# Arieys/MonteCarloPathTracing

Measured on AMD Instinct MI355X. Metric: Mrays/s on cornell-box 1280x720 SPP=256 (closest-hit queries actually traced / wall time incl. gather), higher is better.
Workload: dtype f64

## Files before the change

montecarlopathtracing_amd/csrc/camera.hip:

```cpp
#include <hip/hip_runtime.h>

#include "camera.hpp"
#include "dev_common.hpp"
#include "kernels.hpp"
#include "shade_common.hpp"
#include "shade_path.hpp"
#include "vertex.hpp"
#include "wavefront.hpp"

namespace mcpt {

__global__ void k_primary_pos(DCamera cam, double* __restrict__ pos_out)
{
    const int row = blockIdx.x * blockDim.x + threadIdx.x;
    if (row >= cam.height) return;
    const V3 pdx = ld3(cam.pdx);
    V3 pos = ld3(cam.start_point) - ld3(cam.pdy) * (double)row;
    double* out = pos_out + (size_t)row * cam.width * 3;
    for (int j = 0; j < cam.width; j++) {
        out[j * 3] = pos.x; out[j * 3 + 1] = pos.y; out[j * 3 + 2] = pos.z;
        pos = pos + pdx;
    }
}

// ... 76 lines not shown
    stc(a.out.bdir, cap, j, d);
    a.out.btype[j] = RT_TRANSMISSION | MCPT_BT_NO_OFFSET;
    for (int l = 0; l < a.nl; l++) a.out.expect[(long long)l * cap + j] = -2;
}

template <bool PROG, bool ENV>
__global__ void k_fold_lens(const double* __restrict__ rad, const uint8_t* __restrict__ flags, const int32_t* __restrict__ pixels, int first_slot,
                            int n_slots, int n, int k0, int N, double* __restrict__ img, double* __restrict__ mom, uint8_t* __restrict__ hit,
                            int32_t* __restrict__ hitcnt)
{
    const long long gid = (long long)blockIdx.x * blockDim.x + threadIdx.x;
    if (gid >= (long long)n_slots * 3) return;
    const int s = (int)(gid / 3), c = (int)(gid % 3);
    const int slot = first_slot + s;
    const int pix = pixels ? pixels[slot] : slot;
    const double* src = rad + (size_t)s * n * 3 + c;
    const uint8_t* f = flags + (size_t)s * n;
    int h = 0;
    for (int k = 0; k < n; k++) h += f[k];
    const size_t i = (size_t)pix * 3 + c;
    if (!PROG) {
        float acc = 0.0f;
        if (h > 0 || ENV)
            for (int k = 0; k < n; k++) acc = (float)((double)acc + src[(size_t)k * 3] / n);
        img[i] = (double)acc;
        return;
    }
    if (c == 0) {
        const int total = (k0 > 0 ? hitcnt[pix] : 0) + h;
        hitcnt[pix] = total;
        hit[pix] = total > 0 ? 1 : 0;
    }
    double* m = mom + (size_t)pix * 6 + c;
    if (h == 0 && !ENV) {
        if (k0 == 0) { img[i] = 0.0; m[0] = 0.0; m[3] = 0.0; }
        return;
    }
    float acc = k0 > 0 ? (float)img[i] : 0.0f;
    double s1 = k0 > 0 ? m[0] : 0.0, s2 = k0 > 0 ? m[3] : 0.0;
    for (int k = 0; k < n; k++) {
        const double x = src[(size_t)k * 3];
        acc = (float)((double)acc + x / N);
        s1 += x;
        s2 += x * x;
    }
    img[i] = (double)acc;
    m[0] = s1; m[3] = s2;
}

template <bool ENV>
__global__ void k_fold_motion(const double* __restrict__ rad, const int32_t* __restrict__ pixels, const PrimaryHit* __restrict__ hits, int first_slot,
                              int n_slots, int n, int k0, int N, double* __restrict__ img, double* __restrict__ mom, uint8_t* __restrict__ hit, DEnv env,
                              const double* __restrict__ dirs)
{
    const long long gid = (long long)blockIdx.x * blockDim.x + threadIdx.x;
    if (gid >= (long long)n_slots * 3) return;
    const int s = (int)(gid / 3), c = (int)(gid % 3);
    const int slot = first_slot + s;
    const int pix = pixels ? pixels[slot] : slot;
    const bool h = hits[slot].leaf >= 0;
    if (c == 0) hit[pix] = (uint8_t)((k0 > 0 ? hit[pix] : 0) | (h ? 1 : 0));
    const size_t i = (size_t)pix * 3 + c;
    double* m = mom + (size_t)pix * 6 + c;
    double le = 0.0;
    if (!h) {
        if (ENV) {
            const V3 e = env_eval(env, ld3(dirs + (size_t)pix * 3));
            le = c == 0 ? e.x : (c == 1 ? e.y : e.z);
        } else {
            if (k0 == 0) { img[i] = 0.0; m[0] = 0.0; m[3] = 0.0; }
            return;
        }
    }
    const double* src = rad + (size_t)s * n * 3 + c;
    float acc = k0 > 0 ? (float)img[i] : 0.0f;
    double s1 = k0 > 0 ? m[0] : 0.0, s2 = k0 > 0 ? m[3] : 0.0;
    for (int k = 0; k < n; k++) {
        const double x = h ? src[(size_t)k * 3] : le;
        acc = (float)((double)acc + x / N);
        s1 += x;
        s2 += x * x;
    }
    img[i] = (double)acc;
    m[0] = s1; m[3] = s2;
}

static inline unsigned blocks_of(long long n, int block) { return (unsigned)((n + block - 1) / block); }

void launch_primary_pos(const DCamera& cam, double* d_pos, hipStream_t st)
{
    hipLaunchKernelGGL(k_primary_pos, dim3(blocks_of(cam.height, 64)), dim3(64), 0, st, cam, d_pos);
}
void launch_camera_rays(const DLens& lens, unsigned long long seed, const int32_t* d_pix, const int32_t* d_k, long long n, double* d_rays6, hipStream_t st)
{
    if (n <= 0) return;
    hipLaunchKernelGGL(k_camera_rays, dim3(blocks_of(n, 256)), dim3(256), 0, st, lens, seed, d_pix, d_k, n, d_rays6);
}
void launch_shade_samples_lens(const DScene& S, const DLens& lens, unsigned long long seed, const int32_t* d_pixels, int first_slot, int n_slots, int spp,
                               int sample_base, double* d_rad, uint8_t* d_flags, DCounters* ctr, hipStream_t st)
{
    const long long n = (long long)n_slots * spp;
    if (n <= 0) return;
    const dim3 grid(blocks_of(n, 256));
    with_path_variant(S, [&](auto env, auto pick) {
        hipLaunchKernelGGL((k_shade_samples_lens<env(), pick()>), grid, dim3(256), 0, st, S, lens, seed, d_pixels, first_slot, n, spp, sample_base, d_rad, d_flags, ctr);
// ... 40 lines not shown
```

montecarlopathtracing_amd/csrc/dev_common.hpp:

```cpp
#pragma once
#include <hip/hip_runtime.h>

#include "device_scene.hpp"

namespace mcpt {

#define MCPT_PI 3.1415926
#define MCPT_P_RR 0.6

struct V3 { double x, y, z; };
__device__ __forceinline__ V3 mk(double x, double y, double z) { V3 r; r.x = x; r.y = y; r.z = z; return r; }
__device__ __forceinline__ V3 ld3(const double* p) { return mk(p[0], p[1], p[2]); }
__device__ __forceinline__ V3 operator+(V3 a, V3 b) { return mk(a.x + b.x, a.y + b.y, a.z + b.z); }
__device__ __forceinline__ V3 operator-(V3 a, V3 b) { return mk(a.x - b.x, a.y - b.y, a.z - b.z); }
__device__ __forceinline__ V3 operator*(V3 a, double t) { return mk(a.x * t, a.y * t, a.z * t); }
__device__ __forceinline__ V3 operator/(V3 a, double m) { return mk(a.x / m, a.y / m, a.z / m); }
__device__ __forceinline__ V3 mul(V3 a, V3 b) { return mk(a.x * b.x, a.y * b.y, a.z * b.z); }
__device__ __forceinline__ V3 neg(V3 a) { return mk(-a.x, -a.y, -a.z); }
__device__ __forceinline__ double dot(V3 a, V3 b) { return a.x * b.x + a.y * b.y + a.z * b.z; }
__device__ __forceinline__ V3 cross(V3 a, V3 b) { return mk(a.y * b.z - b.y * a.z, b.x * a.z - a.x * b.z, a.x * b.y - b.x * a.y); }
__device__ __forceinline__ double norm(V3 a) { return sqrt(a.x * a.x + a.y * a.y + a.z * a.z); }
__device__ __forceinline__ V3 normalized(V3 a) { double d = norm(a); return mk(a.x / d, a.y / d, a.z / d); }

__device__ __forceinline__ V3 ldc(const double* __restrict__ a, long long cap, long long i)
// ... 166 lines not shown
    for (int off = 32; off > 0; off >>= 1) { unsigned int o = __shfl_down(v, off, 64); v = o > v ? o : v; }
    return v;
}
struct LaneStats { uint32_t nodes = 0, tris = 0, shadow = 0, bounce = 0, primary = 0, shades = 0, samples = 0, depth = 0, skipped = 0; };
__device__ __forceinline__ void flush_stats(DCounters* c, const LaneStats& s)
{
    if (!c) return;
    const unsigned long long n = wave_sum(s.nodes), t = wave_sum(s.tris), sh = wave_sum(s.shadow), bo = wave_sum(s.bounce),
                             pr = wave_sum(s.primary), sc = wave_sum(s.shades), sa = wave_sum(s.samples), sk = wave_sum(s.skipped);
    const unsigned int md = wave_max(s.depth);
    if ((threadIdx.x & 63) == 0) {
        if (n) atomicAdd(&c->node_visits, n);
        if (t) atomicAdd(&c->tri_tests, t);
        if (sh) atomicAdd(&c->rays_shadow, sh);
        if (bo) atomicAdd(&c->rays_bounce, bo);
        if (pr) atomicAdd(&c->rays_primary, pr);
        if (sc) atomicAdd(&c->shade_calls, sc);
        if (sa) atomicAdd(&c->samples, sa);
        if (sk) atomicAdd(&c->shadow_skipped, sk);
        if (md) atomicMax(&c->max_depth, (unsigned long long)md);
    }
}


}
```

montecarlopathtracing_amd/csrc/kernels.hip:

```cpp
#include <hip/hip_runtime.h>

#include "accel_build.hpp"
#include "dev_common.hpp"
#include "kernels.hpp"
#include "shade_common.hpp"
#include "shade_path.hpp"
#include "trace_persistent.hpp"
#include "trace_pool.hpp"

namespace mcpt {

template <bool LEAF>
__global__ void __launch_bounds__(256) k_trace_closest_reference(DScene S, const double* __restrict__ rays, long long n,
                                                       int32_t* __restrict__ face, double* __restrict__ t_out,
                                                       double* __restrict__ p_out, double* __restrict__ pn_out, DCounters* ctr)
{
    const long long gid = (long long)blockIdx.x * blockDim.x + threadIdx.x;
    LaneStats ls;
    if (gid < n) {
        Ray r;
        r.o = ld3(rays + gid * 6); r.d = ld3(rays + gid * 6 + 3);
        Hit h; Work w = {0, 0};
        const bool ok = trace_closest(S, r, h, w);
        ls.nodes = w.nodes; ls.tris = w.tris; ls.primary = 1;
// ... 196 lines not shown
__global__ void __launch_bounds__(256) k_light_pick_at(DLightPick pick, int nl, unsigned long long seed, const int32_t* __restrict__ pix, const int32_t* __restrict__ ks,
                                                       int depth, const double* __restrict__ p, const double* __restrict__ pn, long long n,
                                                       int32_t* __restrict__ light, double* __restrict__ pdf)
{
    const long long gid = (long long)blockIdx.x * blockDim.x + threadIdx.x;
    if (gid >= n) return;
    RngKey key; key.k0 = (uint32_t)seed; key.k1 = (uint32_t)(seed >> 32); key.pixel = (uint32_t)pix[gid]; key.sample = (uint32_t)ks[gid];
    double q;
    light[gid] = light_pick_at(pick, key, (uint32_t)depth, (uint32_t)nl, ld3(p + gid * 3), ld3(pn + gid * 3), q);
    pdf[gid] = q;
}

template <bool ENV>
__global__ void k_fold_samples(const double* __restrict__ rad, const int32_t* __restrict__ pixels, const PrimaryHit* __restrict__ hits,
                               int first_slot, int n_slots, int spp, double* __restrict__ img, DEnv env, const double* __restrict__ dirs)
{
    const long long gid = (long long)blockIdx.x * blockDim.x + threadIdx.x;
    if (gid >= (long long)n_slots * 3) return;
    const int s = (int)(gid / 3), c = (int)(gid % 3);
    const double* src = rad + (size_t)s * spp * 3 + c;
    const int slot = first_slot + s;
    float acc = 0.0f;
    if (hits[slot].leaf >= 0)
        for (int k = 0; k < spp; k++) acc = (float)((double)acc + src[(size_t)k * 3] / spp);
    else if (ENV) {
        const V3 le = env_eval(env, ld3(dirs + (size_t)(pixels ? pixels[slot] : slot) * 3));
        const double x = c == 0 ? le.x : (c == 1 ? le.y : le.z);
        for (int k = 0; k < spp; k++) acc = (float)((double)acc + x / spp);
    }
    const int pix = pixels ? pixels[slot] : slot;
    img[(size_t)pix * 3 + c] = (double)acc;
}

template <bool ENV>
__global__ void k_fold_progressive(const double* __restrict__ rad, const int32_t* __restrict__ pixels, const PrimaryHit* __restrict__ hits,
                                   int first_slot, int n_slots, int n, int k0, int N, double* __restrict__ img, double* __restrict__ mom,
                                   uint8_t* __restrict__ hit, DEnv env, const double* __restrict__ dirs)
{
    const long long gid = (long long)blockIdx.x * blockDim.x + threadIdx.x;
    if (gid >= (long long)n_slots * 3) return;
    const int s = (int)(gid / 3), c = (int)(gid % 3);
    const int slot = first_slot + s;
    const int pix = pixels ? pixels[slot] : slot;
    const bool h = hits[slot].leaf >= 0;
    if (c == 0) hit[pix] = h ? 1 : 0;
    if (!h) {
        if (ENV) {
            const V3 le = env_eval(env, ld3(dirs + (size_t)pix * 3));
            const double x = c == 0 ? le.x : (c == 1 ? le.y : le.z);
            double* m = mom + (size_t)pix * 6 + c;
            float acc = 0.0f;
            for (int k = 0; k < N; k++) acc = (float)((double)acc + x / N);
            double s1 = k0 > 0 ? m[0] : 0.0;
            for (int k = 0; k < n; k++) s1 += x;
            img[(size_t)pix * 3 + c] = (double)acc;
            m[0] = s1; m[3] = 0.0;
        } else img[(size_t)pix * 3 + c] = 0.0;
        return;
    }
    const double* src = rad + (size_t)s * n * 3 + c;
    double* m = mom + (size_t)pix * 6 + c;
    float acc = k0 > 0 ? (float)img[(size_t)pix * 3 + c] : 0.0f;
    double s1 = k0 > 0 ? m[0] : 0.0, s2 = k0 > 0 ? m[3] : 0.0;
    for (int k = 0; k < n; k++) {
        const double x = src[(size_t)k * 3];
        acc = (float)((double)acc + x / N);
        s1 += x;
        s2 += x * x;
    }
    img[(size_t)pix * 3 + c] = (double)acc;
    m[0] = s1; m[3] = s2;
}

__device__ __forceinline__ double wave_sum_fixed(double v)
{
    for (int o = 32; o >= 1; o >>= 1) v += __shfl_xor(v, o, 64);
    return v;
}
__device__ __forceinline__ void block_sum3(double v[3], double* out)
{
    __shared__ double part[4][3];
    const int w = threadIdx.x >> 6, lane = threadIdx.x & 63;
    for (int i = 0; i < 3; i++) v[i] = wave_sum_fixed(v[i]);
    if (lane == 0) for (int i = 0; i < 3; i++) part[w][i] = v[i];
    __syncthreads();
    if (threadIdx.x == 0)
        for (int i = 0; i < 3; i++) out[i] = ((part[0][i] + part[1][i]) + part[2][i]) + part[3][i];
}
template <bool PER_PIXEL>
__global__ void __launch_bounds__(256) k_noise_reduce(const int32_t* __restrict__ pixels, long long n_pixels, long long per_range,
                                                      const double* __restrict__ mom, const uint8_t* __restrict__ hit, int done,
                                                      const int32_t* __restrict__ cnt, double* __restrict__ partials)
// ... 313 lines not shown
```

montecarlopathtracing_amd/csrc/render.cpp:

```cpp
#include <hip/hip_runtime_api.h>

#include <algorithm>
#include <cmath>
#include <cstdio>
#include <cstring>
#include <functional>
#include <string>
#include <vector>

#include "handles.hpp"

using namespace mcpt;

int ensure_dirs(mcpt_device* d, hipStream_t st)
{
    if (!d->dirs_ready) {
        launch_primary_dirs(d->ds.cam, d->dirs.get(), st);
        HIP_TRY(hipGetLastError());
        HIP_TRY(hipStreamSynchronize(st));
        d->dirs_ready = true;
    }
    return MCPT_OK;
}

// ... 156 lines not shown
    int64_t chunk_slots = std::max<int64_t>(cap / spp, 1);
    chunk_slots = std::min<int64_t>(chunk_slots, npx);
    cap = chunk_slots * spp;
    const size_t ws_need = size_t(cap) * bpp + overhead;
    HIP_TRY(f.wf_ws.grow_bytes(ws_need));
    HIP_TRY(f.rad.grow_bytes(size_t(cap) * 3 * sizeof(double)));
    if (per_sample) {
        HIP_TRY(f.cam_hit.grow(size_t(cap)));
    } else {
        HIP_TRY(f.hit_slots.grow(size_t(chunk_slots)));
        HIP_TRY(f.surf.grow(size_t(chunk_slots)));
        HIP_TRY(f.alive_base.grow(size_t(chunk_slots / 64 + 2)));
    }
    int rc = MCPT_OK;
    WfArgs a{};
    WfState A, B;
    if (!wf_carve(f.wf_ws.get(), f.wf_ws.bytes(), cap, nl, A, B, a.rays)) return fail(MCPT_ERR_NOMEM, "wavefront workspace too small");
    char* path_area = f.path_area.get();
    if (nl != S.num_lights && d->cfg.finish_pool) {
        const size_t need = finish_pool_bytes(d->cfg.cus, nl);
        if (!need) path_area = nullptr;
        else { HIP_TRY(f.path_area.grow_bytes(need)); path_area = f.path_area.get(); }
    }
    a.cap = cap; a.nl = nl; a.spp = spp; a.sample_base = r.k0; a.seed = p->seed; a.pixels = L.pixels; a.hit_slots = f.hit_slots.get(); a.surf = f.surf.get(); a.alive_base = f.alive_base.get();
    a.hits = f.hits.get(); a.dirs = d->dirs.get(); a.rad = f.rad.get(); a.counts = f.wf_counts.get(); a.ctr = f.ctr.get(); a.tris = d->tris.get();
    a.materials = d->materials.get(); a.queue = fast ? f.queue.get() : nullptr;
    a.finish_below = fast ? unsigned(std::min<long long>(std::max<long long>(d->finish_threshold, 0), 1ll << 30)) : 0u;
    if (per_sample) { a.hits = nullptr; a.cam_hit = f.cam_hit.get(); }
    const size_t ev_first = d->ev_used;
    const int kSyncEvery = 4;
    for (int64_t first = 0; first < npx; first += chunk_slots) {
        const int n_slots = int(std::min<int64_t>(chunk_slots, npx - first));
        HIP_TRY(hipMemsetAsync(f.wf_counts.get(), 0, sizeof(WfCounts) * MCPT_WF_COUNT_SLOTS, st));
        long long n_upper = (long long)n_slots * spp;
        double n_grid = double(n_upper);
        a.first_slot = int(first);
        a.in = A; a.out = B;
        a.counts_in = &f.wf_counts[0];
        if (per_sample) {
            WfArgs ac = a;
            ac.depth = -1; ac.counts = &f.wf_counts[0]; ac.count_mul = 1u; ac.finish_below = 0u;
            if (src.query) launch_query_pass(*src.query, ac, n_upper, st);
            else launch_camera_pass(*src.lens, ac, n_upper, st);
            HIP_TRY(hipGetLastError());
            ac.nl = 0;
            EventPair* pr = nullptr;
            if (timed || keep) { if ((rc = next_pair(d->ev_pool, d->ev_used, pr))) return rc; HIP_TRY(hipEventRecord(pr->first.get(), st)); }
// ... 294 lines not shown
```

montecarlopathtracing_amd/csrc/trace_pool.hpp:

```cpp
#pragma once
#include "env.hpp"
#include "trace_persistent.hpp"
#include "vertex.hpp"

namespace mcpt {

struct NoPaths { static constexpr bool kPaths = false; };

#ifndef MCPT_POOL_WAVES
#define MCPT_POOL_WAVES 16
#endif
#ifndef MCPT_POOL_KT
#define MCPT_POOL_KT 20
#endif
#ifndef MCPT_POOL_STACK
#define MCPT_POOL_STACK 8
#endif
#define MCPT_POOL_SPILL (MCPT_FAST_STACK - MCPT_POOL_STACK)
#ifndef MCPT_POOL_CLAIMS
#define MCPT_POOL_CLAIMS 2
#endif
#define MCPT_POOL_CLAIM_ORDER __ATOMIC_ACQUIRE
#define MCPT_POOL_FILE_ORDER __ATOMIC_RELEASE

// ... 427 lines not shown
                }
                const bool want_path = have && mode == P_FREE;
                const unsigned long long wb = __ballot(want_path);
                bool dead = false;
                if (wb) {
                    long long mine = pp.n;
                    if (!queue_empty) {
                        const unsigned int want = (unsigned int)__popcll(wb);
                        unsigned int got = 0;
                        if (lane == 0) got = atomicAdd(&a.counts->finish_claimed, want);
                        got = (unsigned int)uni((int)got);
                        if ((long long)got + want >= pp.n) queue_empty = true;
                        mine = (long long)got + (int)__builtin_amdgcn_mbcnt_hi((unsigned int)(wb >> 32), __builtin_amdgcn_mbcnt_lo((unsigned int)wb, 0u));
                    }
                    if (want_path) {
                        if (mine < pp.n) {
                            const long long j = mine;
                            id = a.out.id[j];
                            depth = (uint32_t)a.depth;
                            T = mk(1, 1, 1); Lr = mk(0, 0, 0);
                            if (folded && a.depth == 0) { const int b0 = a.out.btype[j]; if (b0 >= 0) T = first_vertex_throughput(S, a, id, b0); }
                            else if (a.depth > 0 || folded) T = ldc(a.out.T, cap, j);
                            if (a.depth > 0) Lr = ldc(a.out.L, cap, j);
                            if (a.depth == 0) { const PrimaryHit* ph = a.hits + (a.first_slot + id / a.spp); p = mk(ph->p[0], ph->p[1], ph->p[2]); }
                            else p = ldc(a.out.p, cap, j);
                            for (int l = 0; l < nl; l++) {
                                const int expect = a.out.expect[(long long)l * cap + j];
                                ri[(size_t)(RI_EXPECT + l) * plane] = expect;
                                if (expect != -2) {
                                    const V3 cc = ldc(a.out.c + (long long)l * 3 * cap, cap, j), d = ldc(a.rays.d + (long long)l * 3 * cap, cap, j);
                                    stp(RD_C + 3 * l, cc); emit(s0 + l, p + d * 0.01, d);
                                }
                            }
                            const int bt = a.out.btype[j];
                            ri[RI_BT * plane] = bt;
                            if (bt >= 0) {
                                const V3 bd = ldc(a.out.bdir, cap, j);
                                if (!folded) stp(RD_W, ldc(a.out.w, cap, j));
                                emit(s0 + nl, (bt & MCPT_BT_NO_OFFSET) ? p : p + bd * 0.01, bd);
                            }
                            ri[RI_ID * plane] = id; ri[RI_DEPTH * plane] = (int)depth;
                            stp(RD_T, T); stp(RD_L, Lr);
                            mode = P_ADOPTED;
                        } else dead = true;
                    }
                }
                if (have) {
// ... 143 lines not shown
```

montecarlopathtracing_amd/csrc/vertex.hpp:

```cpp
#pragma once
#include "dev_common.hpp"
#include "shade_common.hpp"
#include "light_tree.hpp"
#include "wavefront.hpp"

namespace mcpt {

__device__ __forceinline__ V3 after_bounce(const V3& T, const V3& wgt)
{
    return mk(T.x * wgt.x * MCPT_INV_P_RR, T.y * wgt.y * MCPT_INV_P_RR, T.z * wgt.z * MCPT_INV_P_RR);
}
__device__ __forceinline__ V3 first_vertex_throughput(const DScene& S, const WfArgs& a, int id, int bt)
{
    const PrimarySurface* ps = a.surf + a.hits[a.first_slot + id / a.spp].surf;
    const int type = bt & 7;
    const V3 wgt = type == RT_DIFFUSE ? ld3(ps->kd) : (type == RT_SPECULAR ? ld3(S.materials[ps->material].ks) : mk(1, 1, 1));
    return after_bounce(mk(1, 1, 1), wgt);
}
__device__ __forceinline__ void add_if_visible(V3& L_dir, const V3& c, bool vis)
{
    L_dir.x += vis ? c.x : c.x * 0.0;
    L_dir.y += vis ? c.y : c.y * 0.0;
    L_dir.z += vis ? c.z : c.z * 0.0;
}
struct PathLights { int nplanes, nlights; bool folded; };
template <bool ENV, int PICK>
__device__ __forceinline__ PathLights path_lights(const DScene& S, int nl)
{
    const int nplanes = ENV ? nl - 1 : nl;
    return {nplanes, PICK ? S.num_lights : nplanes, nl == 1};
}
__device__ __forceinline__ RngKey sample_key(const WfArgs& a, int id, int pixel)
{
    RngKey key;
    key.k0 = (uint32_t)a.seed; key.k1 = (uint32_t)(a.seed >> 32);
    key.pixel = (uint32_t)pixel;
    key.sample = (uint32_t)(a.sample_base + id % a.spp);
    return key;
}
__device__ __forceinline__ RngKey sample_key(const WfArgs& a, int id)
{
    const int slot = a.first_slot + id / a.spp;
    return sample_key(a, id, a.pixels ? a.pixels[slot] : slot);
}

__device__ __forceinline__ void vertex_surface(const DScene& S, int leaf, const V3& p, const DMaterial* m, V3& pn, V3& kd)
{
    const DTri* tr = S.tris + leaf;
    const DTriShade* sh = S.shade + leaf;
    const V3 g = barycentric_s(ld3(tr->v1), ld3(tr->v2), ld3(tr->v3), p);
    pn = (ld3(sh->vn1) * g.x + ld3(sh->vn2) * g.y) + ld3(sh->vn3) * g.z;
    if (m->has_map) {
        const double row = sh->vt1[0] * g.x + sh->vt2[0] * g.y + sh->vt3[0] * g.z;
        const double col = sh->vt1[1] * g.x + sh->vt2[1] * g.y + sh->vt3[1] * g.z;
        const double irow = row - floor(row), icol = col - floor(col);
        int rr = (int)(irow * m->map_h), cc = (int)(icol * m->map_w);
        rr = rr < 0 ? 0 : (rr > m->map_h - 1 ? m->map_h - 1 : rr);
        cc = cc < 0 ? 0 : (cc > m->map_w - 1 ? m->map_w - 1 : cc);
        const uint8_t* px = S.texels + m->tex_offset + ((size_t)rr * m->map_w + cc) * 3;
        kd = mk((double)px[2] * MCPT_INV_255, (double)px[1] * MCPT_INV_255, (double)px[0] * MCPT_INV_255);
    } else kd = ld3(m->kd);
}

__device__ __forceinline__ int light_sample(const DScene& S, const RngKey& key, uint32_t depth, int l, const V3& p, const V3& pn, const V3& kd,
                                            int& sample_mat, V3& direction, V3& c)
{
// ... 114 lines not shown
```

montecarlopathtracing_amd/csrc/wavefront.hpp:

```cpp
#pragma once
#include <hip/hip_runtime_api.h>

#include "device_scene.hpp"
#include "kernels.hpp"

namespace mcpt {

struct WfState {
    int32_t* id;
    double* T;
    double* L;
    double* c;
    int32_t* expect;
    double* w;
    double* bdir;
    int32_t* btype;
    int32_t* hit_mat;
    int32_t* hit_leaf;
    double* p;
};

struct WfRays {
    double* d;
};

struct alignas(16) PrimarySurface {
    double p[3], dir[3];
// ... 26 lines not shown
    WfState in, out;
    WfRays rays;
    long long cap;
    int nl, spp, depth;
    unsigned long long seed;
    const int32_t* pixels;
    const int32_t* hit_slots;
    const PrimarySurface* surf;
    const unsigned int* alive_base;
    PrimaryHit* hits;
    const double* dirs;
    int first_slot;
    double* rad;
    WfCounts* counts;
    const WfCounts* counts_in;
    unsigned int count_mul;
    DCounters* ctr;
    const DTri* tris;
    const DMaterial* materials;
    unsigned int finish_below;
    TraceQueue* queue;
    int sample_base;
    uint8_t* cam_hit;
};

size_t wf_bytes_per_path(int nl);
bool wf_carve(void* base, size_t bytes, long long cap, int nl, WfState& a, WfState& b, WfRays& r);

void launch_wf_logic(const DScene& S, const WfArgs& a, long long n_upper, bool first, hipStream_t st, const LaunchCfg& cfg);
void launch_wf_trace(const DScene& S, const WfArgs& a, long long n_upper, bool fast, TraceQueue* queue, long long* slow_list,
                     unsigned int slow_cap, hipStream_t st, const LaunchCfg& cfg);
void launch_wf_finish(const DScene& S, const WfArgs& a, long long n_upper, hipStream_t st, const LaunchCfg& cfg, char* path_area, long long* slow_list,
                      unsigned int slow_cap);
size_t finish_pool_bytes(int cus, int nl);
int persistent_grid(const void* kernel, int cus);
void init_launch_cfg_logic(LaunchCfg& cfg, unsigned forced_grid);
long long persistent_chunk(long long total, int grid_blocks);

void launch_primary_surface(const DScene& S, const WfArgs& a, PrimarySurface* surf, unsigned int* alive_count, unsigned int* alive_total, int n_slots_upper,
                            hipStream_t st);
void launch_hit_slots(const PrimaryHit* hits, int first_slot, int n_slots, int32_t* hit_slots, unsigned int* count, hipStream_t st);
void launch_zero_rad(double* rad, long long n_doubles, hipStream_t st);
void launch_camera_pass(const DLens& lens, const WfArgs& a, long long n_samples, hipStream_t st);
void launch_query_pass(const DQuery& q, const WfArgs& a, long long n_samples, hipStream_t st);

}
// ... 1 lines not shown
```

montecarlopathtracing_amd/csrc/wavefront_logic.hip:

```cpp
#include <hip/hip_runtime.h>

#include <cstdio>
#include <cstdlib>
#include <cstring>

#include "accel_build.hpp"
#include "dev_common.hpp"
#include "env.hpp"
#include "shade_common.hpp"
#include "trace_persistent.hpp"
#include "trace_pool.hpp"
#include "vertex.hpp"
#include "wave_rank.hpp"
#include "wavefront.hpp"
#include "wf_ray_source.hpp"

namespace mcpt {

#ifndef MCPT_LOGIC_NT
#define MCPT_LOGIC_NT 1
#endif
#if MCPT_LOGIC_NT
template <class T> __device__ __forceinline__ T sld(const T* p) { return __builtin_nontemporal_load(p); }
template <class T> __device__ __forceinline__ void sst(T* p, T v) { __builtin_nontemporal_store(v, p); }
#else
template <class T> __device__ __forceinline__ T sld(const T* p) { return *p; }
template <class T> __device__ __forceinline__ void sst(T* p, T v) { *p = v; }
#endif
__device__ __forceinline__ V3 sldc(const double* __restrict__ a, long long cap, long long i) { return mk(sld(a + i), sld(a + cap + i), sld(a + 2 * cap + i)); }
__device__ __forceinline__ void sstc(double* __restrict__ a, long long cap, long long i, V3 v) { sst(a + i, v.x); sst(a + cap + i, v.y); sst(a + 2 * cap + i, v.z); }

#ifndef MCPT_FINISH_WAVES
#define MCPT_FINISH_WAVES 2
#endif
#ifndef MCPT_LOGIC_WAVES
#define MCPT_LOGIC_WAVES 4
#endif
#ifndef MCPT_LOGIC_WAVES_FIRST
#define MCPT_LOGIC_WAVES_FIRST MCPT_LOGIC_WAVES
#endif

template <bool FIRST, bool ENV, int PICK, class LoadL>
__device__ __forceinline__ void wf_shade_vertex(const DScene& S, const WfArgs& a, long long j_lane, bool ranked, int id, int leaf, const V3& p, const V3& dir, const V3& T,
                                                LoadL load_L, int mat_first, int pix_first, const V3& pn_first, const V3& kd_first, LaneStats& ls)
{
    const long long cap = a.cap;
    const auto [nplanes, nlights, folded] = path_lights<ENV, PICK>(S, a.nl);
    const uint32_t depth = (uint32_t)a.depth;
    const DMaterial* m = S.materials + (FIRST ? mat_first : S.tris[leaf].material);
    V3 pn = pn_first, kd = kd_first;
    if (!FIRST) vertex_surface(S, leaf, p, m, pn, kd);

    const RngKey key = FIRST ? sample_key(a, id, pix_first) : sample_key(a, id);

    long long j = j_lane;
    {
        V3 nd = mk(0, 0, 0), wgt = mk(1, 1, 1);
        const int btype = bounce_sample(key, depth, nlights, m, dir, pn, kd, nd, wgt);
        if (ranked) { const int lane = threadIdx.x & 63; j = j_lane - lane + (long long)bounce_first_rank(__ballot(btype >= 0), lane); }
        sst(a.out.id + j, id);
        if (!FIRST) { sstc(a.out.L, cap, j, load_L()); sstc(a.out.p, cap, j, p); }
        if (btype >= 0) { sstc(a.out.bdir, cap, j, nd); ls.bounce++; }
        sst(a.out.btype + j, btype);
        if (folded) { if (!FIRST && btype >= 0) sstc(a.out.T, cap, j, after_bounce(T, wgt)); }
        else { sstc(a.out.w, cap, j, wgt); if (!FIRST) sstc(a.out.T, cap, j, T); }
    }

    int sample_mat = -1;
    for (int l = 0; l < nplanes; l++) {
        V3 direction, c;
        const int expect = PICK ? light_sample_one<PICK>(S, key, depth, p, pn, kd, direction, c) : light_sample(S, key, depth, l, p, pn, kd, sample_mat, direction, c);
        if (expect != -2) {
            sstc(a.out.c + (long long)l * 3 * cap, cap, j, folded ? mul(T, c) : c);
            sstc(a.rays.d + (long long)l * 3 * cap, cap, j, direction);
            ls.shadow++;
        } else ls.skipped++;
// ... 17 lines not shown

template <bool FIRST, bool ENV, int PICK>
__global__ void __launch_bounds__(256, FIRST ? MCPT_LOGIC_WAVES_FIRST : MCPT_LOGIC_WAVES) k_wf_logic(DScene S, WfArgs a)
{
    const long long n_prev = (long long)a.counts_in->n_next * a.count_mul;
    if (a.queue && blockIdx.x == 0 && threadIdx.x == 0) { a.queue->head = 0ull; a.queue->slow_count = 0u; a.queue->redo_all = 0u; }
    if (!FIRST && n_prev <= (long long)a.finish_below) return;
    const long long cap = a.cap;
    const int nl = a.nl;
    const bool folded = nl == 1;
    const uint32_t depth = (uint32_t)a.depth;
    const int lane = threadIdx.x & 63, wv = threadIdx.x >> 6;
    LaneStats ls;
#ifdef MCPT_TRACE_DIAG
    unsigned long long dg[4] = {0, 0, 0, 0};
    unsigned long long tl = __builtin_amdgcn_s_memtime();
#define MCPT_LSTAMP(k) { const unsigned long long tn = __builtin_amdgcn_s_memtime(); dg[k] += tn - tl; tl = tn; }
#else
#define MCPT_LSTAMP(k)
#endif
    const long long n_round = (n_prev + 255) / 256 * 256;
    if constexpr (FIRST) {
        if (blockIdx.x == 0 && threadIdx.x == 0) a.counts->n_next = a.counts_in->shaded_pixels * (unsigned int)a.spp;
        for (long long base = (long long)blockIdx.x * 256; base < n_round; base += (long long)gridDim.x * 256) {
            const long long i = base + threadIdx.x;
            if (i >= n_prev) continue;
            const PrimarySurface* ps = a.surf + i / a.spp;
            const int k = (int)(i % a.spp);
            unsigned int an = a.alive_base[(i / a.spp) >> 6] + (unsigned int)ps->alive_index;
            const unsigned int n_alive = a.counts_in->shaded_pixels;
#ifndef MCPT_SHUFFLE_LOG2
#define MCPT_SHUFFLE_LOG2 10
#endif
            constexpr unsigned int kWin = (1u << MCPT_SHUFFLE_LOG2) - 1u;
            if ((an | kWin) < n_alive) an = (an & ~kWin) | ((an & kWin) * 40503u & kWin);
            const long long j = (long long)an * a.spp + k;
            const int id = (ps->slot - a.first_slot) * a.spp + k;
            const int leaf = ps->leaf, mat_first = ps->material, pix_first = ps->pixel;
            const V3 p = ld3(ps->p), dir = ld3(ps->dir), pn_first = ld3(ps->pn), kd_first = ld3(ps->kd);
            ls.samples = 1;
            ls.shades++;
            if (depth > ls.depth) ls.depth = depth;
            const DMaterial* m = S.materials + mat_first;
            if (m->light >= 0) {
                const V3 rad = ld3(S.lights[m->light].radiance);
                a.rad[(size_t)id * 3] = rad.x; a.rad[(size_t)id * 3 + 1] = rad.y; a.rad[(size_t)id * 3 + 2] = rad.z;
                MCPT_LSTAMP(0)
                continue;
            }
            MCPT_LSTAMP(0)
            wf_shade_vertex<true, ENV, PICK>(S, a, j, (a.spp & 63) == 0, id, leaf, p, dir, mk(1, 1, 1), [] { return mk(0, 0, 0); }, mat_first, pix_first, pn_first, kd_first, ls);
            MCPT_LSTAMP(2)
        }
    } else {
        constexpr int kPer = MCPT_LOGIC_PER;
        constexpr unsigned int kRing = 512u * kPer;
        static_assert(kPer == 1 || kPer == 2, "ring size: a power of two");
        __shared__ unsigned int wave_tot[2][kPer][4];
        __shared__ unsigned int block_base[2];
        __shared__ int ring_pos[kRing], ring_leaf[kRing];
        __shared__ double ring_L[3][kRing];
        int turn = 0, bturn = 0;
        unsigned int head = 0, count = 0;
        long long base = (long long)blockIdx.x * 256;
        for (;;) {
            while (count < 256u && base < n_round) {
                long long pos[kPer];
                int id[kPer], bt[kPer], hl[kPer];
                V3 L[kPer], T[kPer], wgt[kPer], L_dir[kPer];
                bool alive[kPer];
#pragma unroll
                for (int u = 0; u < kPer; u++) {
                    pos[u] = base + threadIdx.x;
                    base += (long long)gridDim.x * 256;
                    const long long i = pos[u] < n_prev ? pos[u] : 0;
// ... 68 lines not shown
                }
                count = at - head;
                MCPT_LSTAMP(1)
            }
            if (count == 0u) break;
            const unsigned int m_round = count < 256u ? count : 256u;
            bturn ^= 1;
            if (threadIdx.x == 0) block_base[bturn] = atomicAdd(&a.counts->n_next, m_round);
            __syncthreads();
            MCPT_LSTAMP(1)
            if (threadIdx.x < m_round) {
                const unsigned int s = (head + threadIdx.x) & (kRing - 1u);
                const long long i = ring_pos[s];
                const int leaf = ring_leaf[s];
                const long long j = (long long)block_base[bturn] + threadIdx.x;
                const int id = sld(a.in.id + i);
                const int bt = sld(a.in.btype + i);
                V3 T = mk(1, 1, 1);
                if (folded && depth == 1 && a.hits) T = first_vertex_throughput(S, a, id, bt);
                else if (depth > 1 || (folded && depth > 0)) T = sldc(a.in.T, cap, i);
                if (!folded && depth > 0) T = after_bounce(T, sldc(a.in.w, cap, i));
                const V3 bd = sldc(a.in.bdir, cap, i);
                V3 pv;
                if (depth == 1 && a.hits) { const PrimaryHit* ph = a.hits + (a.first_slot + id / a.spp); pv = mk(ph->p[0], ph->p[1], ph->p[2]); }
                else pv = sldc(a.in.p, cap, i);
                const V3 ro = (bt & MCPT_BT_NO_OFFSET) ? pv : pv + bd * 0.01;
                const DTri* tr = S.tris + leaf;
                const V3 v1 = ld3(tr->v1), n = ld3(tr->n);
                const double t = dot(v1 - ro, n) / dot(n, bd);
                const V3 p = ro + bd * t;
                wf_shade_vertex<false, ENV, PICK>(S, a, j, true, id, leaf, p, neg(bd), T, [&] { return mk(ring_L[0][s], ring_L[1][s], ring_L[2][s]); }, 0, 0, mk(0, 0, 0),
                                                  mk(0, 0, 0), ls);
            }
            head = (head + m_round) & (kRing - 1u);
            count -= m_round;
            MCPT_LSTAMP(2)
        }
    }
#ifdef MCPT_TRACE_DIAG
    if (!FIRST && (threadIdx.x & 63) == 0 && a.ctr) { for (int k = 0; k < 3; k++) atomicAdd(&a.ctr->logic_cycles[k], dg[k]); atomicAdd(&a.ctr->logic_waves, 1ull); }
#endif
    flush_stats(a.ctr, ls);
}

template <bool ENV, int PICK>
__global__ void __launch_bounds__(256, MCPT_FINISH_WAVES) k_wf_finish(DScene S, WfArgs a)
{
    __shared__ int lds_stack[MCPT_FAST_STACK * 256];
    const long long n = a.counts->n_next;
    if (n == 0 || n > (long long)a.finish_below) return;
    const long long cap = a.cap;
    const int nl = a.nl;
    const auto [nplanes, nlights, folded] = path_lights<ENV, PICK>(S, nl);
    const int lane = threadIdx.x & 63;
// ... 357 lines not shown
```

montecarlopathtracing_amd/csrc/wf_ray_source.hpp:

```cpp
#pragma once
#include "dev_common.hpp"
#include "vertex.hpp"
#include "wavefront.hpp"

namespace mcpt {

struct WfRaySource {
    static constexpr bool kWantsPoint = false;
    WfArgs a;
    long long n_paths;
    __device__ __forceinline__ long long total() const { return n_paths * (a.nl + 1); }
    __device__ __forceinline__ void split(long long q, int& l, long long& j) const
    {
        l = 0; j = q;
        while (j >= n_paths) { j -= n_paths; l++; }
    }
    __device__ __forceinline__ V3 vertex(long long j) const
    {
        if (a.depth == 0 && a.hits) {
            const PrimaryHit* ph = a.hits + (a.first_slot + a.out.id[j] / a.spp);
            return mk(ph->p[0], ph->p[1], ph->p[2]);
        }
        return ldc(a.out.p, a.cap, j);
    }
    __device__ __forceinline__ bool fetch(long long q, Ray& r) const
    {
        int l; long long j;
        split(q, l, j);
        const bool bounce = l == a.nl;
        const int flag = bounce ? a.out.btype[j] : a.out.expect[(long long)l * a.cap + j];
        const V3 p = vertex(j);
        r.d = ldc(bounce ? a.out.bdir : a.rays.d + (long long)l * 3 * a.cap, a.cap, j);
        r.o = (bounce && (flag & MCPT_BT_NO_OFFSET)) ? p : p + r.d * 0.01;
        return bounce ? flag >= 0 : flag != -2;
    }
    __device__ __forceinline__ void store(long long q, bool ok, const Hit& h) const
    {
        int l; long long j;
        split(q, l, j);
        if (l == a.nl) {
            int v = -1;
            if (ok) { const int mat = h.mat >= 0 ? h.mat : a.tris[h.leaf].material; v = h.leaf | (a.materials[mat].light >= 0 ? MCPT_HIT_EMITTER : 0); }
            a.out.hit_leaf[j] = v;
// ... 24 lines not shown
#endif
struct WfRaySourceK {
    static constexpr bool kWantsPoint = false;
    WfArgsKernarg ap;
    long long n_paths;
    int nl;
    __device__ __forceinline__ WfArgsKernarg args() const { WfArgsKernarg p = ap; __asm__ volatile("" : "+s"(p)); return p; }
    __device__ __forceinline__ long long total() const { return n_paths * (nl + 1); }
    __device__ __forceinline__ void split(long long q, int& l, long long& j) const
    {
        l = 0; j = q;
        while (j >= n_paths) { j -= n_paths; l++; }
    }
    __device__ __forceinline__ bool fetch(long long q, Ray& r) const
    {
        int l; long long j;
        split(q, l, j);
        const WfArgsKernarg A = args();
        const long long cap = A->cap;
        const bool bounce = l == nl;
        const int flag = bounce ? wf_sld(wf_glob(A->out.btype) + j) : wf_sld(wf_glob(A->out.expect) + ((long long)l * cap + j));
        V3 p;
        if (A->depth == 0 && A->hits) {
            const auto* ph = wf_glob(A->hits) + (A->first_slot + wf_glob(A->out.id)[j] / A->spp);
            p = mk(ph->p[0], ph->p[1], ph->p[2]);
        } else {
            const auto* g = wf_glob(A->out.p);
            p = mk(wf_sld(g + j), wf_sld(g + cap + j), wf_sld(g + 2 * cap + j));
        }
        const auto* d = wf_glob(bounce ? A->out.bdir : A->rays.d + (long long)l * 3 * cap);
        r.d = mk(wf_sld(d + j), wf_sld(d + cap + j), wf_sld(d + 2 * cap + j));
        r.o = (bounce && (flag & MCPT_BT_NO_OFFSET)) ? p : p + r.d * 0.01;
        return bounce ? flag >= 0 : flag != -2;
    }
    __device__ __forceinline__ void store(long long q, bool ok, const Hit& h) const
    {
        int l; long long j;
        split(q, l, j);
        const WfArgsKernarg A = args();
        if (l == nl) {
            int v = -1;
            if (ok) { const int mat = h.mat >= 0 ? h.mat : wf_glob(A->tris)[h.leaf].material; v = h.leaf | (wf_glob(A->materials)[mat].light >= 0 ? MCPT_HIT_EMITTER : 0); }
            wf_sst(wf_glob_mut(A->out.hit_leaf) + j, v);
        }
        else wf_sst(wf_glob_mut(A->out.hit_mat) + ((long long)l * A->cap + j), ok ? (h.mat >= 0 ? h.mat : wf_glob(A->tris)[h.leaf].material) : -1);
    }
};
// ... 3 lines not shown
```

Baseline: 5420.

## Replace runtime spp division with precomputed magic-multiply and wave-uniform first-vertex path

Precomputes a magic multiplier for dividing by spp on the host and uses it in place of integer division and modulo by spp in the wavefront kernels. When spp is a power of two, the per-sample 1/N fold uses a reciprocal multiply instead of a divide. The first-vertex shading loop gains a wave-uniform specialization, used when spp is a multiple of 64 and no environment light is present. That path treats the surface, light index and alive counters as scalar values so they can be loaded once per wave. This adds template complexity and relies on the correctness of the magic-division formula for all ids.

```diff
diff --git a/montecarlopathtracing_amd/csrc/camera.hip b/montecarlopathtracing_amd/csrc/camera.hip
--- a/montecarlopathtracing_amd/csrc/camera.hip
+++ b/montecarlopathtracing_amd/csrc/camera.hip
@@ -122,7 +122,7 @@
     if (!PROG) {
         float acc = 0.0f;
         if (h > 0 || ENV)
-            for (int k = 0; k < n; k++) acc = (float)((double)acc + src[(size_t)k * 3] / n);
+            fold_over(n, [&](auto over) { for (int k = 0; k < n; k++) acc = (float)((double)acc + over(src[(size_t)k * 3])); });
         img[i] = (double)acc;
         return;
     }
@@ -138,12 +138,14 @@
     }
     float acc = k0 > 0 ? (float)img[i] : 0.0f;
     double s1 = k0 > 0 ? m[0] : 0.0, s2 = k0 > 0 ? m[3] : 0.0;
-    for (int k = 0; k < n; k++) {
-        const double x = src[(size_t)k * 3];
-        acc = (float)((double)acc + x / N);
-        s1 += x;
-        s2 += x * x;
-    }
+    fold_over(N, [&](auto over) {
+        for (int k = 0; k < n; k++) {
+            const double x = src[(size_t)k * 3];
+            acc = (float)((double)acc + over(x));
+            s1 += x;
+            s2 += x * x;
+        }
+    });
     img[i] = (double)acc;
     m[0] = s1; m[3] = s2;
 }
@@ -175,12 +177,14 @@
     const double* src = rad + (size_t)s * n * 3 + c;
     float acc = k0 > 0 ? (float)img[i] : 0.0f;
     double s1 = k0 > 0 ? m[0] : 0.0, s2 = k0 > 0 ? m[3] : 0.0;
-    for (int k = 0; k < n; k++) {
-        const double x = h ? src[(size_t)k * 3] : le;
-        acc = (float)((double)acc + x / N);
-        s1 += x;
-        s2 += x * x;
-    }
+    fold_over(N, [&](auto over) {
+        for (int k = 0; k < n; k++) {
+            const double x = h ? src[(size_t)k * 3] : le;
+            acc = (float)((double)acc + over(x));
+            s1 += x;
+            s2 += x * x;
+        }
+    });
     img[i] = (double)acc;
     m[0] = s1; m[3] = s2;
 }
diff --git a/montecarlopathtracing_amd/csrc/dev_common.hpp b/montecarlopathtracing_amd/csrc/dev_common.hpp
--- a/montecarlopathtracing_amd/csrc/dev_common.hpp
+++ b/montecarlopathtracing_amd/csrc/dev_common.hpp
@@ -212,5 +212,10 @@
     }
 }
 
-
-}
+template <class Body> __device__ __forceinline__ void fold_over(int N, Body body)
+{
+    if ((N & (N - 1)) == 0) { const double r = 1.0 / (double)N; body([r](double x) { return x * r; }); }
+    else { const double d = (double)N; body([d](double x) { return x / d; }); }
+}
+
+}
diff --git a/montecarlopathtracing_amd/csrc/kernels.hip b/montecarlopathtracing_amd/csrc/kernels.hip
--- a/montecarlopathtracing_amd/csrc/kernels.hip
+++ b/montecarlopathtracing_amd/csrc/kernels.hip
@@ -242,11 +242,11 @@
     const int slot = first_slot + s;
     float acc = 0.0f;
     if (hits[slot].leaf >= 0)
-        for (int k = 0; k < spp; k++) acc = (float)((double)acc + src[(size_t)k * 3] / spp);
+        fold_over(spp, [&](auto over) { for (int k = 0; k < spp; k++) acc = (float)((double)acc + over(src[(size_t)k * 3])); });
     else if (ENV) {
         const V3 le = env_eval(env, ld3(dirs + (size_t)(pixels ? pixels[slot] : slot) * 3));
         const double x = c == 0 ? le.x : (c == 1 ? le.y : le.z);
-        for (int k = 0; k < spp; k++) acc = (float)((double)acc + x / spp);
+        fold_over(spp, [&](auto over) { for (int k = 0; k < spp; k++) acc = (float)((double)acc + over(x)); });
     }
     const int pix = pixels ? pixels[slot] : slot;
     img[(size_t)pix * 3 + c] = (double)acc;
@@ -270,7 +270,7 @@
             const double x = c == 0 ? le.x : (c == 1 ? le.y : le.z);
             double* m = mom + (size_t)pix * 6 + c;
             float acc = 0.0f;
-            for (int k = 0; k < N; k++) acc = (float)((double)acc + x / N);
+            fold_over(N, [&](auto over) { for (int k = 0; k < N; k++) acc = (float)((double)acc + over(x)); });
             double s1 = k0 > 0 ? m[0] : 0.0;
             for (int k = 0; k < n; k++) s1 += x;
             img[(size_t)pix * 3 + c] = (double)acc;
@@ -282,12 +282,14 @@
     double* m = mom + (size_t)pix * 6 + c;
     float acc = k0 > 0 ? (float)img[(size_t)pix * 3 + c] : 0.0f;
     double s1 = k0 > 0 ? m[0] : 0.0, s2 = k0 > 0 ? m[3] : 0.0;
-    for (int k = 0; k < n; k++) {
-        const double x = src[(size_t)k * 3];
-        acc = (float)((double)acc + x / N);
-        s1 += x;
-        s2 += x * x;
-    }
+    fold_over(N, [&](auto over) {
+        for (int k = 0; k < n; k++) {
+            const double x = src[(size_t)k * 3];
+            acc = (float)((double)acc + over(x));
+            s1 += x;
+            s2 += x * x;
+        }
+    });
     img[(size_t)pix * 3 + c] = (double)acc;
     m[0] = s1; m[3] = s2;
 }
diff --git a/montecarlopathtracing_amd/csrc/render.cpp b/montecarlopathtracing_amd/csrc/render.cpp
--- a/montecarlopathtracing_amd/csrc/render.cpp
+++ b/montecarlopathtracing_amd/csrc/render.cpp
@@ -202,7 +202,7 @@
         if (!need) path_area = nullptr;
         else { HIP_TRY(f.path_area.grow_bytes(need)); path_area = f.path_area.get(); }
     }
-    a.cap = cap; a.nl = nl; a.spp = spp; a.sample_base = r.k0; a.seed = p->seed; a.pixels = L.pixels; a.hit_slots = f.hit_slots.get(); a.surf = f.surf.get(); a.alive_base = f.alive_base.get();
+    a.cap = cap; a.nl = nl; a.spp = spp; a.spp_div = spp_div_make(uint32_t(spp)); a.sample_base = r.k0; a.seed = p->seed; a.pixels = L.pixels; a.hit_slots = f.hit_slots.get(); a.surf = f.surf.get(); a.alive_base = f.alive_base.get();
     a.hits = f.hits.get(); a.dirs = d->dirs.get(); a.rad = f.rad.get(); a.counts = f.wf_counts.get(); a.ctr = f.ctr.get(); a.tris = d->tris.get();
     a.materials = d->materials.get(); a.queue = fast ? f.queue.get() : nullptr;
     a.finish_below = fast ? unsigned(std::min<long long>(std::max<long long>(d->finish_threshold, 0), 1ll << 30)) : 0u;
diff --git a/montecarlopathtracing_amd/csrc/spp_div.hpp b/montecarlopathtracing_amd/csrc/spp_div.hpp
--- /dev/null
+++ b/montecarlopathtracing_amd/csrc/spp_div.hpp
@@ -0,0 +1,40 @@
+#pragma once
+#include <stdint.h>
+
+#if defined(__HIPCC__) || defined(__CUDACC__)
+#define MCPT_SPP_DIV_FN __host__ __device__ inline
+#else
+#define MCPT_SPP_DIV_FN inline
+#endif
+
+namespace mcpt {
+
+struct SppDiv {
+    uint32_t d;
+    uint32_t m;
+    uint32_t l;
+};
+
+MCPT_SPP_DIV_FN SppDiv spp_div_make(uint32_t d)
+{
+    SppDiv s;
+    s.d = d;
+    s.l = 0;
+    while ((uint64_t(1) << s.l) < d) s.l++;
+    s.m = (uint32_t)(((uint64_t(1) << (31 + s.l)) + d - 1) / d);
+    return s;
+}
+MCPT_SPP_DIV_FN uint32_t spp_div(const SppDiv& s, uint32_t n)
+{
+    return (uint32_t)(((uint64_t)(n << 1) * s.m) >> 32) >> s.l;
+}
+MCPT_SPP_DIV_FN uint32_t spp_mod(const SppDiv& s, uint32_t n, uint32_t q)
+{
+    return n - q * s.d;
+}
+MCPT_SPP_DIV_FN uint32_t spp_mod(const SppDiv& s, uint32_t n)
+{
+    return spp_mod(s, n, spp_div(s, n));
+}
+
+}
diff --git a/montecarlopathtracing_amd/csrc/trace_pool.hpp b/montecarlopathtracing_amd/csrc/trace_pool.hpp
--- a/montecarlopathtracing_amd/csrc/trace_pool.hpp
+++ b/montecarlopathtracing_amd/csrc/trace_pool.hpp
@@ -473,7 +473,7 @@
                             if (folded && a.depth == 0) { const int b0 = a.out.btype[j]; if (b0 >= 0) T = first_vertex_throughput(S, a, id, b0); }
                             else if (a.depth > 0 || folded) T = ldc(a.out.T, cap, j);
                             if (a.depth > 0) Lr = ldc(a.out.L, cap, j);
-                            if (a.depth == 0) { const PrimaryHit* ph = a.hits + (a.first_slot + id / a.spp); p = mk(ph->p[0], ph->p[1], ph->p[2]); }
+                            if (a.depth == 0) { const PrimaryHit* ph = a.hits + (a.first_slot + (int)spp_div(a.spp_div, (uint32_t)id)); p = mk(ph->p[0], ph->p[1], ph->p[2]); }
                             else p = ldc(a.out.p, cap, j);
                             for (int l = 0; l < nl; l++) {
                                 const int expect = a.out.expect[(long long)l * cap + j];
diff --git a/montecarlopathtracing_amd/csrc/vertex.hpp b/montecarlopathtracing_amd/csrc/vertex.hpp
--- a/montecarlopathtracing_amd/csrc/vertex.hpp
+++ b/montecarlopathtracing_amd/csrc/vertex.hpp
@@ -12,7 +12,7 @@
 }
 __device__ __forceinline__ V3 first_vertex_throughput(const DScene& S, const WfArgs& a, int id, int bt)
 {
-    const PrimarySurface* ps = a.surf + a.hits[a.first_slot + id / a.spp].surf;
+    const PrimarySurface* ps = a.surf + a.hits[a.first_slot + (int)spp_div(a.spp_div, (uint32_t)id)].surf;
     const int type = bt & 7;
     const V3 wgt = type == RT_DIFFUSE ? ld3(ps->kd) : (type == RT_SPECULAR ? ld3(S.materials[ps->material].ks) : mk(1, 1, 1));
     return after_bounce(mk(1, 1, 1), wgt);
@@ -30,18 +30,19 @@
     const int nplanes = ENV ? nl - 1 : nl;
     return {nplanes, PICK ? S.num_lights : nplanes, nl == 1};
 }
-__device__ __forceinline__ RngKey sample_key(const WfArgs& a, int id, int pixel)
+__device__ __forceinline__ RngKey sample_key(const WfArgs& a, int k, int pixel)
 {
     RngKey key;
     key.k0 = (uint32_t)a.seed; key.k1 = (uint32_t)(a.seed >> 32);
     key.pixel = (uint32_t)pixel;
-    key.sample = (uint32_t)(a.sample_base + id % a.spp);
+    key.sample = (uint32_t)(a.sample_base + k);
     return key;
 }
 __device__ __forceinline__ RngKey sample_key(const WfArgs& a, int id)
 {
-    const int slot = a.first_slot + id / a.spp;
-    return sample_key(a, id, a.pixels ? a.pixels[slot] : slot);
+    const uint32_t q = spp_div(a.spp_div, (uint32_t)id);
+    const int slot = a.first_slot + (int)q;
+    return sample_key(a, (int)spp_mod(a.spp_div, (uint32_t)id, q), a.pixels ? a.pixels[slot] : slot);
 }
 
 __device__ __forceinline__ void vertex_surface(const DScene& S, int leaf, const V3& p, const DMaterial* m, V3& pn, V3& kd)
diff --git a/montecarlopathtracing_amd/csrc/wavefront.hpp b/montecarlopathtracing_amd/csrc/wavefront.hpp
--- a/montecarlopathtracing_amd/csrc/wavefront.hpp
+++ b/montecarlopathtracing_amd/csrc/wavefront.hpp
@@ -3,6 +3,7 @@
 
 #include "device_scene.hpp"
 #include "kernels.hpp"
+#include "spp_div.hpp"
 
 namespace mcpt {
 
@@ -75,6 +76,7 @@
     TraceQueue* queue;
     int sample_base;
     uint8_t* cam_hit;
+    SppDiv spp_div;
 };
 
 size_t wf_bytes_per_path(int nl);
diff --git a/montecarlopathtracing_amd/csrc/wavefront_logic.hip b/montecarlopathtracing_amd/csrc/wavefront_logic.hip
--- a/montecarlopathtracing_amd/csrc/wavefront_logic.hip
+++ b/montecarlopathtracing_amd/csrc/wavefront_logic.hip
@@ -3,6 +3,7 @@
 #include <cstdio>
 #include <cstdlib>
 #include <cstring>
+#include <type_traits>
 
 #include "accel_build.hpp"
 #include "dev_common.hpp"
@@ -42,7 +43,7 @@
 
 template <bool FIRST, bool ENV, int PICK, class LoadL>
 __device__ __forceinline__ void wf_shade_vertex(const DScene& S, const WfArgs& a, long long j_lane, bool ranked, int id, int leaf, const V3& p, const V3& dir, const V3& T,
-                                                LoadL load_L, int mat_first, int pix_first, const V3& pn_first, const V3& kd_first, LaneStats& ls)
+                                                LoadL load_L, int mat_first, int pix_first, int k_first, const V3& pn_first, const V3& kd_first, LaneStats& ls)
 {
     const long long cap = a.cap;
     const auto [nplanes, nlights, folded] = path_lights<ENV, PICK>(S, a.nl);
@@ -51,7 +52,7 @@
     V3 pn = pn_first, kd = kd_first;
     if (!FIRST) vertex_surface(S, leaf, p, m, pn, kd);
 
-    const RngKey key = FIRST ? sample_key(a, id, pix_first) : sample_key(a, id);
+    const RngKey key = FIRST ? sample_key(a, k_first, pix_first) : sample_key(a, id);
 
     long long j = j_lane;
     {
@@ -115,35 +116,55 @@
     const long long n_round = (n_prev + 255) / 256 * 256;
     if constexpr (FIRST) {
         if (blockIdx.x == 0 && threadIdx.x == 0) a.counts->n_next = a.counts_in->shaded_pixels * (unsigned int)a.spp;
-        for (long long base = (long long)blockIdx.x * 256; base < n_round; base += (long long)gridDim.x * 256) {
-            const long long i = base + threadIdx.x;
-            if (i >= n_prev) continue;
-            const PrimarySurface* ps = a.surf + i / a.spp;
-            const int k = (int)(i % a.spp);
-            unsigned int an = a.alive_base[(i / a.spp) >> 6] + (unsigned int)ps->alive_index;
-            const unsigned int n_alive = a.counts_in->shaded_pixels;
 #ifndef MCPT_SHUFFLE_LOG2
 #define MCPT_SHUFFLE_LOG2 10
 #endif
+        const auto first_vertex = [&](auto uni_tag, long long i) {
+            constexpr bool UNI = decltype(uni_tag)::value;
+            typedef const PrimarySurface __attribute__((address_space(4)))* SurfK;
+            uint32_t pn, k;
+            if constexpr (UNI) {
+                const uint32_t i0 = (uint32_t)uni((int)(i - lane));
+                pn = spp_div(a.spp_div, i0);
+                k = spp_mod(a.spp_div, i0, pn) + (uint32_t)lane;
+            } else {
+                pn = spp_div(a.spp_div, (uint32_t)i);
+                k = spp_mod(a.spp_div, (uint32_t)i, pn);
+            }
+            const PrimarySurface* psg = a.surf + pn;
+            const auto ps = [&] { if constexpr (UNI) return (SurfK)(unsigned long long)psg; else return psg; }();
+            unsigned int an = a.alive_base[pn >> 6] + (unsigned int)ps->alive_index;
+            unsigned int n_alive = a.counts_in->shaded_pixels;
+            if constexpr (UNI) { an = (unsigned int)uni((int)an); n_alive = (unsigned int)uni((int)n_alive); }
             constexpr unsigned int kWin = (1u << MCPT_SHUFFLE_LOG2) - 1u;
             if ((an | kWin) < n_alive) an = (an & ~kWin) | ((an & kWin) * 40503u & kWin);
             const long long j = (long long)an * a.spp + k;
-            const int id = (ps->slot - a.first_slot) * a.spp + k;
+            const int id = (ps->slot - a.first_slot) * a.spp + (int)k;
             const int leaf = ps->leaf, mat_first = ps->material, pix_first = ps->pixel;
-            const V3 p = ld3(ps->p), dir = ld3(ps->dir), pn_first = ld3(ps->pn), kd_first = ld3(ps->kd);
+            const V3 p = mk(ps->p[0], ps->p[1], ps->p[2]), dir = mk(ps->dir[0], ps->dir[1], ps->dir[2]);
+            const V3 pn_first = mk(ps->pn[0], ps->pn[1], ps->pn[2]), kd_first = mk(ps->kd[0], ps->kd[1], ps->kd[2]);
             ls.samples = 1;
             ls.shades++;
             if (depth > ls.depth) ls.depth = depth;
             const DMaterial* m = S.materials + mat_first;
-            if (m->light >= 0) {
-                const V3 rad = ld3(S.lights[m->light].radiance);
+            int light = m->light;
+            if constexpr (UNI) light = uni(light);
+            if (light >= 0) {
+                const V3 rad = ld3(S.lights[light].radiance);
                 a.rad[(size_t)id * 3] = rad.x; a.rad[(size_t)id * 3 + 1] = rad.y; a.rad[(size_t)id * 3 + 2] = rad.z;
                 MCPT_LSTAMP(0)
-                continue;
+                return;
             }
             MCPT_LSTAMP(0)
-            wf_shade_vertex<true, ENV, PICK>(S, a, j, (a.spp & 63) == 0, id, leaf, p, dir, mk(1, 1, 1), [] { return mk(0, 0, 0); }, mat_first, pix_first, pn_first, kd_first, ls);
+            wf_shade_vertex<true, ENV, PICK>(S, a, j, UNI || (a.spp & 63) == 0, id, leaf, p, dir, mk(1, 1, 1), [] { return mk(0, 0, 0); }, mat_first, pix_first, (int)k, pn_first, kd_first, ls);
             MCPT_LSTAMP(2)
+        };
+        const bool whole_waves = !ENV && (a.spp & 63) == 0;
+        for (long long base = (long long)blockIdx.x * 256; base < n_round; base += (long long)gridDim.x * 256) {
+            const long long i = base + threadIdx.x;
+            if (i >= n_prev) continue;
+            if constexpr (!ENV) { if (whole_waves) { first_vertex(std::true_type(), i); continue; } }
+            first_vertex(std::false_type(), i);
         }
     } else {
         constexpr int kPer = MCPT_LOGIC_PER;
@@ -258,14 +279,14 @@
                 if (!folded && depth > 0) T = after_bounce(T, sldc(a.in.w, cap, i));
                 const V3 bd = sldc(a.in.bdir, cap, i);
                 V3 pv;
-                if (depth == 1 && a.hits) { const PrimaryHit* ph = a.hits + (a.first_slot + id / a.spp); pv = mk(ph->p[0], ph->p[1], ph->p[2]); }
+                if (depth == 1 && a.hits) { const PrimaryHit* ph = a.hits + (a.first_slot + (int)spp_div(a.spp_div, (uint32_t)id)); pv = mk(ph->p[0], ph->p[1], ph->p[2]); }
                 else pv = sldc(a.in.p, cap, i);
                 const V3 ro = (bt & MCPT_BT_NO_OFFSET) ? pv : pv + bd * 0.01;
                 const DTri* tr = S.tris + leaf;
                 const V3 v1 = ld3(tr->v1), n = ld3(tr->n);
                 const double t = dot(v1 - ro, n) / dot(n, bd);
                 const V3 p = ro + bd * t;
-                wf_shade_vertex<false, ENV, PICK>(S, a, j, true, id, leaf, p, neg(bd), T, [&] { return mk(ring_L[0][s], ring_L[1][s], ring_L[2][s]); }, 0, 0, mk(0, 0, 0),
+                wf_shade_vertex<false, ENV, PICK>(S, a, j, true, id, leaf, p, neg(bd), T, [&] { return mk(ring_L[0][s], ring_L[1][s], ring_L[2][s]); }, 0, 0, 0, mk(0, 0, 0),
                                                   mk(0, 0, 0), ls);
             }
             head = (head + m_round) & (kRing - 1u);
diff --git a/montecarlopathtracing_amd/csrc/wf_ray_source.hpp b/montecarlopathtracing_amd/csrc/wf_ray_source.hpp
--- a/montecarlopathtracing_amd/csrc/wf_ray_source.hpp
+++ b/montecarlopathtracing_amd/csrc/wf_ray_source.hpp
@@ -18,7 +18,7 @@
     __device__ __forceinline__ V3 vertex(long long j) const
     {
         if (a.depth == 0 && a.hits) {
-            const PrimaryHit* ph = a.hits + (a.first_slot + a.out.id[j] / a.spp);
+            const PrimaryHit* ph = a.hits + (a.first_slot + (int)spp_div(a.spp_div, (uint32_t)a.out.id[j]));
             return mk(ph->p[0], ph->p[1], ph->p[2]);
         }
         return ldc(a.out.p, a.cap, j);
@@ -89,7 +89,8 @@
         const int flag = bounce ? wf_sld(wf_glob(A->out.btype) + j) : wf_sld(wf_glob(A->out.expect) + ((long long)l * cap + j));
         V3 p;
         if (A->depth == 0 && A->hits) {
-            const auto* ph = wf_glob(A->hits) + (A->first_slot + wf_glob(A->out.id)[j] / A->spp);
+            const SppDiv sd = {A->spp_div.d, A->spp_div.m, A->spp_div.l};
+            const auto* ph = wf_glob(A->hits) + (A->first_slot + (int)spp_div(sd, (uint32_t)wf_glob(A->out.id)[j]));
             p = mk(ph->p[0], ph->p[1], ph->p[2]);
         } else {
             const auto* g = wf_glob(A->out.p);
```

Result: no change. 5459 (median of 2 runs) (+0.7%).
